# zdule/distributed_learning

Hardware: AMD Instinct MI355X
Metric: images/sec (whole node) ResNet-50 synthetic ImageNet (higher is better)
Workload: dtype bf16

## Files before the change

### csrc/include/dla_kernels.h

```cpp
#pragma once

#include <hip/hip_runtime.h>
#include <stdint.h>

namespace dla {

enum DType : int { kF32 = 0, kBF16 = 1 };

struct SgdEntry {
  float* param;
  const void* grad;
  float* momentum;
  uint16_t* param_bf16;
  int64_t numel;
};

struct SgdParams {
  float lr;
  float momentum;
  float dampening;
  float weight_decay;
  float grad_scale;
  int nesterov;
  int first_step;
// ... 136 lines not shown
                        hipStream_t stream);
void launch_bn_bwd(const void* dy, const void* y, const uint8_t* mask, const void* x, void* dx, void* dres,
                   int64_t M, int C, int dtype, const float* gamma, float* ws, float* part, float* dgamma,
                   float* dbeta, int mask_mode, hipStream_t stream, const float* ext_part = nullptr,
                   int ext_nrb = 0, int64_t ld_dy = 0);

constexpr int kMaxBnGroups = 4;
struct BnGroups {
  int n;
  int begin[kMaxBnGroups + 1];
  const uint16_t* x[kMaxBnGroups];
  uint16_t* y[kMaxBnGroups];
  const uint16_t* dy[kMaxBnGroups];
  int64_t ldy[kMaxBnGroups], lddy[kMaxBnGroups];
  int64_t ldx[kMaxBnGroups], lddx[kMaxBnGroups];
  int ldp[kMaxBnGroups];
  int C[kMaxBnGroups], tpr[kMaxBnGroups], nrb[kMaxBnGroups];
  const float* part[kMaxBnGroups];
  float* wpart[kMaxBnGroups];
  const float* gamma[kMaxBnGroups];
  const float* beta[kMaxBnGroups];
  float* rm[kMaxBnGroups];
  float* rv[kMaxBnGroups];
  float* ws[kMaxBnGroups];
  float eps[kMaxBnGroups], mom[kMaxBnGroups];
  uint16_t* dx[kMaxBnGroups];
  float* dgamma[kMaxBnGroups];
  float* dbeta[kMaxBnGroups];
};
int bn_group_bwd_rows(int64_t M, const int* C, int n);
void launch_bn_group_fwd(BnGroups G, int64_t M, hipStream_t stream);
void launch_bn_group_bwd(BnGroups G, bool ext, int64_t M, hipStream_t stream);

void launch_bn_relu_maxpool_fwd(const void* x, const float* ws, void* y, uint8_t* pos, int N, int H, int W, int C,
                                int OH, int OW, int k, int s, int p, hipStream_t stream);
void launch_bn_relu_maxpool_bwd(const void* dy_pool, const uint8_t* pos, const void* x, void* dx, int N, int H, int W,
                                int C, int OH, int OW, int k, int s, int p, const float* gamma, float* ws, float* part,
                                float* dgamma, float* dbeta, hipStream_t stream);

void launch_maxpool_fwd(const void* x, void* y, uint8_t* pos, int N, int H, int W, int C, int OH, int OW, int k,
                        int s, int p, int dtype, hipStream_t stream);
void launch_maxpool_bwd(const void* dy, const uint8_t* pos, void* dx, int N, int H, int W, int C, int OH, int OW,
                        int k, int s, int p, int dtype, hipStream_t stream);
bool pool_fast_index(int64_t work, int64_t d0, int64_t d1, int64_t d2);
void set_pool3_sep(int rows);
int pool3_strip_rows();
void launch_gap_fwd(const void* x, void* y, int N, int HW, int C, int dtype, hipStream_t stream);
void launch_subsample2(const void* x, void* y, int N, int H, int W, int C, hipStream_t stream);
void launch_gap_bwd(const void* dy, void* dx, int N, int HW, int C, int dtype, hipStream_t stream);

void set_mfma_pipeline(int p);
int mfma_pipeline();
int mfma_pipeline_for(int K);
enum TileCfg : int {
  kTileAuto = 0,
  kTile128x128 = 1,
  kTile128x64 = 2,
  kTile64x64 = 3,
  kTile256x128 = 4,
  kTile256x128w4 = 5,
  kTile128x256w4 = 6,
  kTile256x64 = 7,
  kTile256x256 = 8,
  kTile512x128 = 9
};
int pick_tile(int64_t M, int N, int tile, int K = 0, bool wide_ok = true, bool stats = false);
void set_tile256_min_k_stats(int k);
bool tile256_enabled();
bool tn256_enabled();
inline int tile_bm(int cfg) {
  if (cfg == kTile512x128) return 512;
  return cfg == kTile64x64 ? 64
                           : ((cfg == kTile256x128 || cfg == kTile256x128w4 || cfg == kTile256x64 || cfg == kTile256x256)
                                  ? 256
                                  : 128);
}
inline int tile_bn(int cfg) {
  if (cfg == kTile512x128) return 128;
  return (cfg == kTile128x256w4 || cfg == kTile256x256) ? 256
                                                       : ((cfg == kTile128x128 || cfg == kTile256x128 || cfg == kTile256x128w4) ? 128 : 64);
}
int gemm_nt_stats_rows(int M, int N, int tile = kTileAuto, int K = 0, bool stats_fwd = true);
void set_tile256_min_k(int k);
int gemm_stream_rows(int64_t M, int N, int K, int64_t lda, int64_t ldc, bool b_kmajor, bool add = false,
                     bool bnb = false);
struct BnBwdArgs;
bool launch_gemm_stream(const void* A, int64_t lda, const void* B, int64_t ldb, bool b_kmajor, void* C, int64_t ldc,
                        int M, int N, int K, float* stats, hipStream_t stream, const void* addend = nullptr,
                        int64_t ldd = 0, const uint8_t* addend_mask = nullptr, const BnBwdArgs* bn_bwd = nullptr,
                        const float* apply_ws = nullptr, void* apply_out = nullptr);
void set_gemm_stream(int mode);
bool gemm_direct_ok(int N, int64_t ldc, const void* addend, int64_t ldd);
void launch_gemm_direct(const void* A, int64_t lda, const void* B, int64_t ldb, bool b_kmajor, void* C, int64_t ldc,
                        int M, int N, int K, float* stats, const void* addend, int64_t ldd,
                        const uint8_t* addend_mask, hipStream_t stream);
void set_gemm_direct(int mode);
constexpr int kGemmApplyMaxK = 2048;
bool gemm_apply_ok(int64_t M, int N, int K);
void set_gemm_apply_max_k(int k);
void set_gemm256_direct(int mode);
bool gemm256_direct_enabled();
void set_wgrad_w4(int mode);
int gemm_apply_rows(int64_t M);
void launch_gemm_apply(const void* y, const void* r, const float* ws, const float* ws2, void* out, uint8_t* mask,
                       const void* B, int64_t ldb, void* C, int M, int N, int K, float* stats, hipStream_t stream,
                       void* xs = nullptr, int H = 0, int W = 0);
// ... 83 lines not shown
```

### csrc/include/dla_mfma.h

```cpp
#pragma once

#include "dla_common.h"

namespace dla {
namespace mm {

typedef __bf16 bf16x8_t __attribute__((ext_vector_type(8)));
typedef float f32x4_t __attribute__((ext_vector_type(4)));
typedef short s16x4_t __attribute__((ext_vector_type(4)));

struct FastDiv {
  uint32_t d, m_lo, m_hi;
};
__host__ __device__ inline FastDiv make_fastdiv(uint32_t d) {
  const uint64_t m = ((1ull << 40) + d - 1) / d;
  return FastDiv{d, (uint32_t)m, (uint32_t)(m >> 32)};
}
__device__ __forceinline__ uint32_t fdiv(uint32_t n, const FastDiv& f) {
  return (__umulhi(n, f.m_lo) + n * f.m_hi) >> 8;
}

constexpr int kThreads = 256;
#ifndef DLA_RM_SWIZZLE
#define DLA_RM_SWIZZLE 1
#endif
#ifndef DLA_EPI_SWZ
#define DLA_EPI_SWZ 1
#endif

constexpr int kBK = 64;

#ifndef DLA_EPI_PRELOAD
#define DLA_EPI_PRELOAD 1
#endif
#ifndef DLA_TR_CONCAT
#define DLA_TR_CONCAT 1
#endif

__host__ __device__ constexpr int blocks_per_cu(int BM, int BN, int NT) {
  return (NT == kThreads && BM * BN <= 128 * 128) ? 2 : 1;
}

__device__ __forceinline__ f32x4_t mfma16(const bf16x8_t& a, const bf16x8_t& b, const f32x4_t& c) {
  return __builtin_amdgcn_mfma_f32_16x16x32_bf16(a, b, c, 0, 0, 0);
}

#ifndef DLA_MFMA_SHAPE
#define DLA_MFMA_SHAPE 16
#endif
constexpr int kMS = DLA_MFMA_SHAPE;
constexpr int kKS = 512 / kMS;
constexpr int kAccN = kMS * kMS / 64;
static_assert(kMS == 16 || kMS == 32, "MFMA shape 16 or 32");
// ... 480 lines not shown
    loader_step(pa, k0, 0);
    const uint32_t a_base = lds0 + (uint32_t)((t % NS) * (SA + SB)) * 2u + wofs;
#pragma unroll
    for (int i = 0; i < GA::CH; ++i) glds16(loader_src(pa, i, k0, 0), a_base + (uint32_t)(i * NT * 16));
  };
  auto issue_b = [&](int t) {
    const int k0 = kbeg + t * kBK;
    loader_step(pb, k0, 0);
    const uint32_t b_base = lds0 + (uint32_t)((t % NS) * (SA + SB) + SA) * 2u + wofs;
#pragma unroll
    for (int i = 0; i < GB::CH; ++i) glds16(loader_src(pb, i, k0, 0), b_base + (uint32_t)(i * NT * 16));
  };
#pragma unroll
  for (int p = 0; p < NS - 1; ++p)
    if (p < nk) {
      issue_a(p);
      issue_b(p);
    }
  for (int t = 0; t < nk; ++t) {
    if constexpr (NS == 3) {
      if (t + 1 < nk) vm_wait<L>();
      else vm_wait<0>();
    } else {
      vm_wait<0>();
    }
    asm volatile("s_waitcnt lgkmcnt(0)" ::: "memory");
    __builtin_amdgcn_s_barrier();
    asm volatile("" ::: "memory");
    const bool more = t + NS - 1 < nk;
    if (more) issue_a(t + NS - 1);
    const bf16_t* As = base + (t % NS) * (SA + SB);
    const bf16_t* Bs = As + SA;
    kstep_mfma<BM, BN, NT, LA, LB, kT>(As, Bs, wr, wc, acc, [&] {
      if (more) issue_b(t + NS - 1);
    });
  }
  __syncthreads();
}

template <class L, int W, int NT>
__device__ __forceinline__ void bissue(const L& l, int k0, uint32_t lds) {
  constexpr int CH = TileGeom<W, NT>::CH;
  uint32_t vo[CH];
  if (l.bcheck(k0)) {
#pragma unroll
    for (int i = 0; i < CH; ++i) vo[i] = l.bvoff_chk(i, k0);
  } else {
#pragma unroll
    for (int i = 0; i < CH; ++i) vo[i] = l.bvo[i];
  }
  bglds<CH, NT * 16>(vo, l.bsrd, (uint32_t)__builtin_amdgcn_readfirstlane(l.bsoff(k0)), lds);
}

template <int BM, int BN, int NT, int NS, bool kT = false, class LA, class LB>
__device__ __forceinline__ void mainloop_bglds(const LA& la, const LB& lb, int kbeg, int kend, Acc<BM, BN, NT>& acc,
                                               char* smem) {
  static_assert(NS == 2 || NS == 3, "2 or 3 stages");
  static_assert(LA::kNT == NT && LB::kNT == NT, "loaders built for another block size");
  using GA = TileGeom<BM, NT>;
  using GB = TileGeom<BN, NT>;
  using AC = Acc<BM, BN, NT>;
  constexpr int L = GA::CH + GB::CH;
  constexpr int WM = AC::WM, WN = AC::WN, TM = AC::TM, TN = AC::TN;
  constexpr int SA = BM * kBK, SB = BN * kBK;
  bf16_t* base = reinterpret_cast<bf16_t*>(smem);
  const int wave = threadIdx.x >> 6, wr = wave / AC::WGN, wc = wave % AC::WGN;
  const uint32_t lds0 = lds_addr(smem);
  const uint32_t wofs = (uint32_t)__builtin_amdgcn_readfirstlane(wave * 64 * 16);
  const int nk = (kend - kbeg + kBK - 1) / kBK;
  if (nk <= 0) return;
  LA pa = la;
  LB pb = lb;
  pa.prep();
  pb.prep();
  pa.bprep();
  pb.bprep();
  auto issue_a = [&](int t) {
    const int k0 = kbeg + t * kBK;
    loader_step(pa, k0, 0);
    bissue<LA, BM, NT>(pa, k0, lds0 + (uint32_t)((t % NS) * (SA + SB)) * 2u + wofs);
  };
  auto issue_b = [&](int t) {
    const int k0 = kbeg + t * kBK;
    loader_step(pb, k0, 0);
    bissue<LB, BN, NT>(pb, k0, lds0 + (uint32_t)((t % NS) * (SA + SB) + SA) * 2u + wofs);
  };
#pragma unroll
  for (int p = 0; p < NS - 1; ++p)
    if (p < nk) {
      issue_a(p);
      issue_b(p);
    }
  for (int t = 0; t < nk; ++t) {
    if constexpr (NS == 3) {
      if (t + 1 < nk) vm_wait<L>();
      else vm_wait<0>();
    } else {
      vm_wait<0>();
    }
    asm volatile("s_waitcnt lgkmcnt(0)" ::: "memory");
    __builtin_amdgcn_s_barrier();
    asm volatile("" ::: "memory");
    const bool more = t + NS - 1 < nk;
    if (more) issue_a(t + NS - 1);
    const bf16_t* As = base + (t % NS) * (SA + SB);
    const bf16_t* Bs = As + SA;
    kstep_mfma<BM, BN, NT, LA, LB, kT>(As, Bs, wr, wc, acc, [&] {
      if (more) issue_b(t + NS - 1);
    });
  }
  __syncthreads();
}

template <int PIPE, bool kT = false, int BM, int BN, int NT, class LA, class LB>
__device__ __forceinline__ void run_mainloop(const LA& la, const LB& lb, int kbeg, int kend, Acc<BM, BN, NT>& acc,
                                             char* smem) {
  if constexpr (PIPE == 0) mainloop<BM, BN, NT, kT>(la, lb, kbeg, kend, acc, smem);
  else if constexpr (PIPE >= 6) mainloop_bglds<BM, BN, NT, PIPE - 4, kT>(la, lb, kbeg, kend, acc, smem);
  else if constexpr (PIPE >= 4) mainloop_glds2<BM, BN, NT, PIPE - 2, kT>(la, lb, kbeg, kend, acc, smem);
  else mainloop_glds<BM, BN, NT, PIPE, kT>(la, lb, kbeg, kend, acc, smem);
}

template <int PIPE, int BM, int BN, class LA, class LB>
__host__ __device__ constexpr size_t run_mainloop_lds_bytes() {
  return PIPE == 0 ? mainloop_lds_bytes<BM, BN, LA, LB>()
                   : glds_lds_bytes<BM, BN, (PIPE >= 6 ? PIPE - 4 : (PIPE >= 4 ? PIPE - 2 : PIPE))>();
}

template <int BM, int BN, bool kStats, int NT = kThreads>
__host__ __device__ constexpr size_t epilogue_lds_bytes() {
  return (size_t)BM * (BN + 8) * sizeof(bf16_t) > (size_t)NT * 64 ? (size_t)BM * (BN + 8) * sizeof(bf16_t)
                                                                  : (size_t)NT * 64;
}

template <int BM, int BN, int NT = kThreads>
struct ColStats {
  float s[Acc<BM, BN, NT>::TN], q[Acc<BM, BN, NT>::TN];
  __device__ void zero() {
#pragma unroll
    for (int j = 0; j < Acc<BM, BN, NT>::TN; ++j) s[j] = q[j] = 0.f;
  }
};

struct BnBwdEpi {
  const bf16_t* x;
  int64_t ldx;
  const float* ws;
  const uint8_t* mask;
  int mode;
  float* part;
  const uint8_t* dmask;
  const bf16_t* d2;
  int H, W;
  FastDiv fW, fH;
};

struct RowIdent {
  __device__ __forceinline__ int64_t operator()(int64_t gm) const { return gm; }
};

template <int BM, int BN, bool kStats, bool kEpi = false, int NT = kThreads, class RM = RowIdent>
__device__ __forceinline__ void epilogue_bf16(const Acc<BM, BN, NT>& acc, bf16_t* __restrict__ C, int64_t ldc,
                                              int64_t M, int N, int64_t row0, int col0, ColStats<BM, BN, NT>& st,
                                              const bf16_t* __restrict__ D, int64_t ldd, char* smem,
                                              const BnBwdEpi* epi = nullptr, int bm = 0, RM rowmap = RM()) {
  const BnBwdEpi* bnb = (kEpi && epi && epi->x) ? epi : nullptr;
  const uint8_t* __restrict__ dmask = (kEpi && epi) ? epi->dmask : nullptr;
  const bf16_t* __restrict__ d2 = (kEpi && epi) ? epi->d2 : nullptr;
  using AC = Acc<BM, BN, NT>;
  constexpr int WM = AC::WM, WN = AC::WN, TM = AC::TM, TN = AC::TN;
  static_assert(!DLA_EPI_SWZ || BN >= 32, "the staging XOR needs 4 chunks per row");
  constexpr int LDS_C = DLA_EPI_SWZ ? BN : BN + 8;
  auto cs_off = [](int m, int n) {
    if constexpr (DLA_EPI_SWZ) return m * BN + ((((n >> 3) ^ (((m >> 2) & 1) << 1))) << 3) + (n & 7);
    else return m * (BN + 8) + n;
  };
  (void)LDS_C;
  const int tid = threadIdx.x, lane = tid & 63, wid = tid >> 6, wr = wid / AC::WGN, wc = wid % AC::WGN,
            fr = acc_col(lane);
// ... 342 lines not shown
```

### csrc/kernels/conv.hip

```cpp
#include "dla_common.h"
#include "dla_kernels.h"
#include "dla_knob.h"
#include "dla_mfma.h"

#include <algorithm>
#include <cstdlib>
#include <type_traits>

namespace dla {

using namespace mm;

struct ConvGeom {
  int N, H, W, Cin;
  int OH, OW, Cout;
  int stride;
  FastDiv fOW, fOH;
};

template <int W, bool kFlip, int NT = kThreads>
struct Im2colRowLoader {
  static constexpr bool kKMajor = false;
  static constexpr int kNT = NT;
  static constexpr int CH = TileGeom<W, NT>::CH;
// ... 517 lines not shown
  const int tile = lin % ntiles, split = lin / ntiles;
  const int bm = tile / nbn, bn = tile % nbn;
  const int kbeg = split * k_per_split;
  const int kend = min(P, kbeg + k_per_split);
  const int m0 = bm * BM, n0 = bn * BN;
  const KLoader<BM, NT> la{dy, g.Cout, m0, Mo, kend};
  Im2colKLoader<BN, PIPE != 0, NT> lb{x, g, kend};
  lb.init(n0);
  Acc<BM, BN, NT> acc;
  acc.zero();
  run_mainloop<PIPE>(la, lb, kbeg, kend, acc, smem_raw);
  epilogue_f32<BM, BN, NT>(acc, part + (int64_t)split * Mo * No, Mo, No, m0, n0);
}

static int conv_pipeline(int K, int deep) {
  const int forced = mfma_pipeline();
  if (forced >= 0) return forced;
  static Knob k_conv_pipe = Knob::integer("CONV_PIPE", -1);
  const int env = k_conv_pipe.value();
  return K >= 256 ? (env >= 0 ? env : deep) : 0;
}

static ConvGeom make_geom(int N, int H, int W, int Cin, int Cout, int stride) {
  ConvGeom g;
  g.N = N;
  g.H = H;
  g.W = W;
  g.Cin = Cin;
  g.Cout = Cout;
  g.stride = stride;
  g.OH = (H + 2 - 3) / stride + 1;
  g.OW = (W + 2 - 3) / stride + 1;
  g.fOW = make_fastdiv((uint32_t)g.OW);
  g.fOH = make_fastdiv((uint32_t)g.OH);
  return g;
}

template <int BM, int BN, bool S, int PIPE, int NT>
static void launch_fwd_p(const bf16_t* x, const bf16_t* w, bf16_t* y, const ConvGeom& g, float* stats,
                         hipStream_t stream) {
  const int64_t P = (int64_t)g.N * g.OH * g.OW;
  const int tiles = (int)((P + BM - 1) / BM) * ((g.Cout + BN - 1) / BN);
  const size_t lds =
      std::max(run_mainloop_lds_bytes<PIPE % 100, BM, BN, Im2colRowLoader<BM, false, NT>, RowLoader<BN, NT>>(),
               epilogue_lds_bytes<BM, BN, S, NT>());
  hipLaunchKernelGGL((conv3x3_fwd_kernel<BM, BN, S, PIPE, NT>), dim3(tiles), dim3(NT), lds, stream, x, w, y, g,
                     stats);
}
template <int BM, int BN, bool S, int NTW = kThreads>
static void launch_fwd(const bf16_t* x, const bf16_t* w, bf16_t* y, const ConvGeom& g, float* stats,
                       hipStream_t stream) {
  if constexpr (NTW == 512 && BM * BN > 256 * 128) {
    if (mfma_pipeline() == 2) launch_fwd_p<BM, BN, S, 2, 512>(x, w, y, g, stats, stream);
    else launch_fwd_p<BM, BN, S, 6, 512>(x, w, y, g, stats, stream);
  } else if constexpr (NTW == 512) {
    if (mfma_pipeline() == 7) launch_fwd_p<BM, BN, S, 7, 512>(x, w, y, g, stats, stream);
    else launch_fwd_p<BM, BN, S, 3, 512>(x, w, y, g, stats, stream);
  } else if constexpr (BM * BN > 128 * 128) {
    if (mfma_pipeline() == 2) launch_fwd_p<BM, BN, S, 2, kThreads>(x, w, y, g, stats, stream);
    else launch_fwd_p<BM, BN, S, 3, kThreads>(x, w, y, g, stats, stream);
  } else if (g.Cin % 64 != 0) {
    if (mfma_pipeline_for(9 * g.Cin) == 0) launch_fwd_p<BM, BN, S, 100, kThreads>(x, w, y, g, stats, stream);
    else launch_fwd_p<BM, BN, S, 102, kThreads>(x, w, y, g, stats, stream);
  } else {
    switch (conv_pipeline(9 * g.Cin, 6)) {
      case 0: launch_fwd_p<BM, BN, S, 0, kThreads>(x, w, y, g, stats, stream); break;
      case 3: launch_fwd_p<BM, BN, S, 3, kThreads>(x, w, y, g, stats, stream); break;
      case 4: launch_fwd_p<BM, BN, S, 4, kThreads>(x, w, y, g, stats, stream); break;
      case 6: launch_fwd_p<BM, BN, S, 6, kThreads>(x, w, y, g, stats, stream); break;
      default: launch_fwd_p<BM, BN, S, 2, kThreads>(x, w, y, g, stats, stream); break;
    }
  }
}

static Knob k_tile512 = Knob::on_unless_0("TILE512");
static bool tile512_enabled() { return k_tile512.on(); }

int pick_conv_tile(int64_t P, int N, int tile, int K, bool wide_ok) {
  if (tile == kTileAuto && wide_ok && tile256_enabled() && tile512_enabled() && N == 128 && K >= 1024 &&
      (P + 511) / 512 >= 1024)
    return kTile512x128;
  return pick_tile(P, N, tile, K, wide_ok);
}

int conv3x3_stats_rows(int64_t P, int Cout, int tile, int K, bool wide_ok) {
  const int bm = tile_bm(pick_conv_tile(P, Cout, tile, K, wide_ok));
  return (int)((P + bm - 1) / bm);
}

void launch_conv3x3_fwd(const void* x, const void* w, void* y, int N, int H, int W, int Cin, int Cout, int stride,
                        float* stats, hipStream_t stream, int tile) {
  if (tile == kTileAuto && halo_conv_eligible(Cin, Cout, W, stride, true)) {
    launch_conv3x3_halo(x, w, y, N, H, W, stats, stream);
    return;
  }
  const ConvGeom g = make_geom(N, H, W, Cin, Cout, stride);
  const bf16_t* xp = (const bf16_t*)x;
  const bf16_t* wp = (const bf16_t*)w;
  bf16_t* yp = (bf16_t*)y;
#define DLA_CFW(BM_, BN_, NT_)                                                  \
  if (stats) launch_fwd<BM_, BN_, true, NT_>(xp, wp, yp, g, stats, stream);   \
  else launch_fwd<BM_, BN_, false, NT_>(xp, wp, yp, g, stats, stream);
#define DLA_CF(BM_, BN_) DLA_CFW(BM_, BN_, kThreads)
  switch (pick_conv_tile((int64_t)g.N * g.OH * g.OW, Cout, tile, 9 * Cin, Cin % 64 == 0)) {
    case kTile512x128: DLA_CFW(512, 128, 512) break;
    case kTile256x256: DLA_CFW(256, 256, 512) break;
// ... 180 lines not shown
```

### csrc/kernels/gemm.hip

```cpp
#include <cstdlib>
#include <type_traits>

#include "dla_common.h"
#include "dla_kernels.h"
#include "dla_knob.h"
#include "dla_mfma.h"

namespace dla {

using namespace mm;

template <int BM, int BN, bool kStats, bool kBT, int PIPE, int NT, bool kD = false>
__global__ __launch_bounds__(NT, blocks_per_cu(BM, BN, NT)) void gemm_nt_kernel(const bf16_t* __restrict__ A, int64_t lda,
                                                              const bf16_t* __restrict__ B, int64_t ldb,
                                                              bf16_t* __restrict__ C, int64_t ldc, int M, int N, int K,
                                                              float* __restrict__ stats, const bf16_t* __restrict__ D,
                                                              int64_t ldd, BnBwdEpi bnb) {
  extern __shared__ __attribute__((aligned(16))) char smem_raw[];
  const int nbn = (N + BN - 1) / BN;
  const int tile = xcd_remap(blockIdx.x, gridDim.x);
  const int bm = tile / nbn, bn = tile % nbn;
  const int64_t row0 = (int64_t)bm * BM;
  const int col0 = bn * BN;
  ColStats<BM, BN, NT> st;
// ... 97 lines not shown
    }
  }
}

template <typename T, int SG>
__global__ __launch_bounds__(256) void splitk_reduce_sg_kernel(const float* __restrict__ P, int splits, int64_t n,
                                                               T* __restrict__ out, float scale, int accumulate,
                                                               const bf16_t* __restrict__ D, int64_t ldd, int ncol) {
  auto addend = [&](int64_t i) -> float {
    if (D == nullptr) return 0.f;
    const int64_t r = i / ncol;
    return bf16_to_f32(D[r * ldd + (i - r * ncol)]);
  };
  constexpr int kOpb = 256 / SG;
  __shared__ float4_t red[SG][kOpb];
  const int g = threadIdx.x / kOpb, o = threadIdx.x % kOpb;
  const int64_t nv = n / 4;
  const int64_t v = (int64_t)blockIdx.x * kOpb + o;
  float4_t a0{0.f, 0.f, 0.f, 0.f}, a1 = a0;
  if (v < nv) {
    int k = g;
    for (; k + SG < splits; k += 2 * SG) {
      a0 += reinterpret_cast<const float4_t*>(P + (int64_t)k * n)[v];
      a1 += reinterpret_cast<const float4_t*>(P + (int64_t)(k + SG) * n)[v];
    }
    if (k < splits) a0 += reinterpret_cast<const float4_t*>(P + (int64_t)k * n)[v];
  }
  red[g][o] = a0 + a1;
  __syncthreads();
  if (g == 0 && v < nv) {
    float4_t s = red[0][o];
#pragma unroll
    for (int j = 1; j < SG; ++j) s += red[j][o];
    s *= scale;
#pragma unroll
    for (int j = 0; j < 4; ++j) {
      float r = s[j] + addend(v * 4 + j);
      if (accumulate) r += Cvt<T>::to_f32(out[v * 4 + j]);
      out[v * 4 + j] = Cvt<T>::from_f32(r);
    }
  }
  if (blockIdx.x == 0) {
    for (int64_t i = nv * 4 + threadIdx.x; i < n; i += blockDim.x) {
      float r = 0.f;
      for (int k = 0; k < splits; ++k) r += P[(int64_t)k * n + i];
      r = r * scale + addend(i);
      if (accumulate) r += Cvt<T>::to_f32(out[i]);
      out[i] = Cvt<T>::from_f32(r);
    }
  }
}

static int g_pipe = -1;
void set_mfma_pipeline(int p) { g_pipe = (p == 0 || (p >= 2 && p <= 7)) ? p : -1; }
int mfma_pipeline() { return g_pipe; }
int mfma_pipeline_for(int K) { return g_pipe >= 0 ? g_pipe : (K >= 256 ? 2 : 0); }

template <int BM, int BN, bool S, bool BT, int PIPE, int NT, bool kD = false>
static void launch_nt_p(const bf16_t* A, int64_t lda, const bf16_t* B, int64_t ldb, bf16_t* C, int64_t ldc, int M,
                        int N, int K, float* stats, const bf16_t* D, int64_t ldd, const BnBwdEpi& bnb,
                        hipStream_t stream) {
  const int tiles = ((M + BM - 1) / BM) * ((N + BN - 1) / BN);
  const size_t ab = BT ? run_mainloop_lds_bytes<PIPE, BM, BN, RowLoader<BM, NT>, KLoader<BN, NT>>()
                       : run_mainloop_lds_bytes<PIPE, BM, BN, RowLoader<BM, NT>, RowLoader<BN, NT>>();
  const size_t cs = epilogue_lds_bytes<BM, BN, S, NT>();
  hipLaunchKernelGGL((gemm_nt_kernel<BM, BN, S, BT, PIPE, NT, kD>), dim3(tiles), dim3(NT), std::max(ab, cs), stream, A,
                     lda, B, ldb, C, ldc, M, N, K, stats, D, ldd, bnb);
}

template <int BM, int BN, bool S, bool BT, int NTW = kThreads>
static void launch_nt(const bf16_t* A, int64_t lda, const bf16_t* B, int64_t ldb, bf16_t* C, int64_t ldc, int M,
                      int N, int K, float* stats, const bf16_t* D, int64_t ldd, const BnBwdEpi& bnb,
                      hipStream_t stream) {
  if constexpr (NTW == 512 && BM * BN > 256 * 128) {
    if (mfma_pipeline() == 2) launch_nt_p<BM, BN, S, BT, 2, 512>(A, lda, B, ldb, C, ldc, M, N, K, stats, D, ldd, bnb, stream);
    else launch_nt_p<BM, BN, S, BT, 6, 512>(A, lda, B, ldb, C, ldc, M, N, K, stats, D, ldd, bnb, stream);
  } else if constexpr (NTW == 512) {
    if (mfma_pipeline() == 7) launch_nt_p<BM, BN, S, BT, 7, 512>(A, lda, B, ldb, C, ldc, M, N, K, stats, D, ldd, bnb, stream);
    else launch_nt_p<BM, BN, S, BT, 3, 512>(A, lda, B, ldb, C, ldc, M, N, K, stats, D, ldd, bnb, stream);
  } else if constexpr (BM * BN > 128 * 128) {
    if (mfma_pipeline() == 2) launch_nt_p<BM, BN, S, BT, 2, kThreads>(A, lda, B, ldb, C, ldc, M, N, K, stats, D, ldd, bnb, stream);
    else launch_nt_p<BM, BN, S, BT, 3, kThreads>(A, lda, B, ldb, C, ldc, M, N, K, stats, D, ldd, bnb, stream);
  } else {
    const int pipe = mfma_pipeline() >= 0 ? mfma_pipeline() : (K > 512 ? 2 : 0);
    switch (pipe) {
      case 0: launch_nt_p<BM, BN, S, BT, 0, kThreads>(A, lda, B, ldb, C, ldc, M, N, K, stats, D, ldd, bnb, stream); break;
      case 3: launch_nt_p<BM, BN, S, BT, 3, kThreads>(A, lda, B, ldb, C, ldc, M, N, K, stats, D, ldd, bnb, stream); break;
      case 4: launch_nt_p<BM, BN, S, BT, 4, kThreads>(A, lda, B, ldb, C, ldc, M, N, K, stats, D, ldd, bnb, stream); break;
      case 6: launch_nt_p<BM, BN, S, BT, 6, kThreads>(A, lda, B, ldb, C, ldc, M, N, K, stats, D, ldd, bnb, stream); break;
      default: launch_nt_p<BM, BN, S, BT, 2, kThreads>(A, lda, B, ldb, C, ldc, M, N, K, stats, D, ldd, bnb, stream); break;
    }
  }
}

static Knob k_tile256 = Knob::on_unless_0("TILE256");
bool tile256_enabled() { return k_tile256.on(); }

static int g_tile256_min_k = 1024;
void set_tile256_min_k(int k) { g_tile256_min_k = k > 0 ? k : 1024; }
static Knob k_tile256_min_k_stats = Knob::positive("TILE256_MIN_K_STATS", 256);
void set_tile256_min_k_stats(int k) { k_tile256_min_k_stats.set(k); }

static Knob k_gemm256_direct = Knob::off_unless_1("GEMM256_DIRECT");
void set_gemm256_direct(int mode) { k_gemm256_direct.set(mode); }
bool gemm256_direct_enabled() { return k_gemm256_direct.on(); }

int pick_tile(int64_t M, int N, int tile, int K, bool wide_ok, bool stats) {
  if (tile != kTileAuto) return tile;
  const int min_k = stats ? std::min(g_tile256_min_k, k_tile256_min_k_stats.value()) : g_tile256_min_k;
  if (wide_ok && tile256_enabled() && K >= min_k && N % 256 == 0 && ((M + 255) / 256) * (N / 256) >= 192)
    return kTile256x256;
  return N <= 64 ? kTile128x64 : kTile128x128;
}

int gemm_nt_stats_rows(int M, int N, int tile, int K, bool stats_fwd) {
  const int bm = tile_bm(pick_tile(M, N, tile, K, true, stats_fwd));
  return (M + bm - 1) / bm;
}

void launch_gemm_nt(const void* A, int64_t lda, const void* B, int64_t ldb, void* C, int64_t ldc, int M, int N, int K,
                    float* stats, hipStream_t stream, const void* addend, int64_t ld_addend, bool b_kmajor, int tile,
                    const BnBwdArgs* bn_bwd, const uint8_t* addend_mask, const void* addend2_s2, int H, int W) {
  BnBwdEpi bnb{};
  if (bn_bwd) {
    bnb.x = (const bf16_t*)bn_bwd->x;
    bnb.ldx = bn_bwd->ldx;
    bnb.ws = bn_bwd->ws;
    bnb.mask = bn_bwd->mask;
// ... 191 lines not shown
```

### csrc/nn_bindings.cpp

```cpp
#include <torch/extension.h>
#include <ATen/hip/HIPContext.h>
#include <c10/hip/HIPStream.h>

#include "dla_bindings.h"
#include "dla_kernels.h"
#include "dla_knob.h"
#include "dla_tables.h"

namespace dla {

static void check_span(const at::Tensor& t, const char* what) {
  int64_t last = 0;
  for (int64_t d = 0; d < t.dim(); ++d) last += (t.size(d) - 1) * t.stride(d);
  const int64_t bytes = t.numel() ? (last + 1) * (int64_t)t.element_size() : 0;
  TORCH_CHECK(bytes < (int64_t(1) << 31), what, ": ", bytes,
              " bytes reach the 2 GiB buffer-descriptor range of the native kernels (lower the per-GPU batch)");
}

static void check_act(const at::Tensor& t, const char* what) {
  TORCH_CHECK(t.is_cuda(), what, " must be a GPU tensor");
  TORCH_CHECK(t.dim() == 4 || t.dim() == 2, what, " must be NCHW-shaped (channels_last) or [M, C]");
  const bool ok = t.dim() == 4 ? t.is_contiguous(at::MemoryFormat::ChannelsLast) : t.is_contiguous();
  TORCH_CHECK(ok, what, " must be channels_last (4-D) or contiguous (2-D)");
  TORCH_CHECK(t.size(1) % 8 == 0, what, ": channel count must be a multiple of 8");
// ... 1025 lines not shown
                         current_stream(dy));
  return dx;
}

std::vector<at::Tensor> conv3x3_dgrad_bn(at::Tensor dy, at::Tensor w, c10::optional<at::Tensor> addend,
                                         at::Tensor x_bn, at::Tensor ws, c10::optional<at::Tensor> mask, int64_t mode) {
  at::Tensor dx = dgrad_dx("conv3x3_dgrad_bn", dy, w);
  const int N = (int)dy.size(0), Cout = (int)w.size(0), Cin = (int)w.size(1), H = (int)dy.size(2), W = (int)dy.size(3);
  const void* add = dgrad_addend("conv3x3_dgrad_bn", addend, dx);
  const int64_t P = (int64_t)N * H * W;
  at::Tensor part;
  const BnBwdArgs bnb = make_bn_bwd("conv3x3_dgrad_bn", x_bn, ws, mask, mode, P, Cin,
                                    conv3x3_stats_rows(P, Cin, kTileAuto, 9 * Cout, Cout % 64 == 0), part);
  launch_conv3x3_dgrad(dy.data_ptr(), w.data_ptr(), dx.data_ptr(), N, H, W, Cin, Cout, add, current_stream(dy),
                       kTileAuto, &bnb);
  return {dx, part};
}

at::Tensor conv3x3_wgrad(at::Tensor dy, at::Tensor x, int64_t stride, c10::ScalarType out_dtype) {
  const int out_code = out_dtype_code(out_dtype, "conv3x3_wgrad");
  dy = dy.contiguous(at::MemoryFormat::ChannelsLast);
  TORCH_CHECK(x.is_cuda() && x.dim() == 4 && x.scalar_type() == at::kBFloat16 &&
                  x.is_contiguous(at::MemoryFormat::ChannelsLast) && x.size(1) % 8 == 0,
              "conv3x3_wgrad: x must be bf16 channels_last with Cin % 8 == 0");
  TORCH_CHECK(dy.is_cuda() && dy.scalar_type() == at::kBFloat16 && dy.size(1) % 8 == 0,
              "conv3x3_wgrad: dy must be a bf16 GPU tensor, Cout % 8");
  TORCH_CHECK(x.numel() / x.size(1) < (1 << 24), "conv3x3_wgrad: too many pixels");
  const int N = (int)x.size(0), Cin = (int)x.size(1), H = (int)x.size(2), W = (int)x.size(3), Cout = (int)dy.size(1);
  TORCH_CHECK(dy.size(2) == (H - 1) / stride + 1 && dy.size(3) == (W - 1) / stride + 1, "conv3x3_wgrad: dy shape");
  at::Tensor dw = at::empty({Cout, Cin, 3, 3}, x.options().dtype(out_dtype).memory_format(at::MemoryFormat::ChannelsLast));
  if (halo_wgrad_eligible(Cin, Cout, W, (int)stride) && (int64_t)N * (H + 2) * (W + 2) < (1 << 30)) {
    const int hs = halo_wgrad_splits(N, H, W);
    at::Tensor hpart = at::empty({(int64_t)hs * Cout * 9 * Cin}, x.options().dtype(at::kFloat));
    launch_conv3x3_halo_wgrad(dy.data_ptr(), x.data_ptr(), hpart.data_ptr<float>(), hs, dw.data_ptr(), out_code, N, H, W,
                              current_stream(x));
    return dw;
  }
  const int splits = conv3x3_wgrad_splits(N, H, W, Cin, Cout, (int)stride);
  at::Tensor part = at::empty({(int64_t)splits * Cout * 9 * Cin}, x.options().dtype(at::kFloat));
  launch_conv3x3_wgrad(dy.data_ptr(), x.data_ptr(), part.data_ptr<float>(), splits, dw.data_ptr(), out_code, N, H, W,
                       Cin, Cout, (int)stride, current_stream(x));
  return dw;
}

void bind_nn(pybind11::module& m) {
  m.def("gemm_nt_bn", &gemm_nt_bn, "gemm_nt producing a fused BN's dy plus its backward-reduction partials",
        pybind11::arg("A"), pybind11::arg("B"), pybind11::arg("addend"), pybind11::arg("b_kmajor"),
        pybind11::arg("x_bn"), pybind11::arg("ws"), pybind11::arg("mask"), pybind11::arg("mode"),
        pybind11::arg("addend_mask") = pybind11::none(), pybind11::arg("addend2") = pybind11::none(),
        pybind11::arg("H") = 0, pybind11::arg("W") = 0);
  m.def("conv3x3_dgrad_bn", &conv3x3_dgrad_bn, "3x3 dgrad producing a fused BN's dy plus its backward partials",
        pybind11::arg("dy"), pybind11::arg("w"), pybind11::arg("addend"), pybind11::arg("x_bn"), pybind11::arg("ws"),
        pybind11::arg("mask"), pybind11::arg("mode"));
  m.def("set_mfma_pipeline", &set_mfma_pipeline, "MFMA main loop: 0 register staging, 2/3 LDS-DMA stages, -1 per-shape auto");
  m.def("set_gemm_stream", &set_gemm_stream, "persistent streaming 1x1 GEMM: -1 environment (default on), 0 off, 1 on");
  m.def("set_gemm_persist", &set_gemm_persist, "persistent register-stored 1x1 GEMM: blocks per CU (0 off, -1 env)");
  m.def("set_gemm_direct", &set_gemm_direct, "register-stored 128x128 1x1 GEMM tiles: -1 environment (default off), 0 / 1");
  m.def("gemm_stream_rows", &gemm_stream_rows, "BN-statistics partial rows of the streaming GEMM (0: shape not served)",
        pybind11::arg("M"), pybind11::arg("N"), pybind11::arg("K"), pybind11::arg("lda"), pybind11::arg("ldc"), pybind11::arg("b_kmajor") = false,
        pybind11::arg("add") = false, pybind11::arg("bnb") = false);
  m.def("mfma_pipeline", &mfma_pipeline);
  m.def("set_tile256_min_k_stats", &set_tile256_min_k_stats, "smallest K of the auto 256x256 tiles of statistics forwards (A/B)");
  m.def("set_tile256_min_k", &set_tile256_min_k, "smallest K of the auto 256x256 gemm_nt / conv tiles (A/B; <= 0 default 1024)");
  m.def("set_tn256", &set_tn256, "256x256 weight-gradient tiles: -1 environment (DLA_TN256, default on), 0 off, 1 on");
  m.def("set_splitk_blocks", &set_splitk_blocks, "split-K weight-gradient block target (0 = default / DLA_SPLITK_BLOCKS)");
  m.def("splitk_target_blocks", &splitk_target_blocks);
  m.def("set_bn_red_blocks", &set_bn_red_blocks, "BN reduction-pass block target (0 = default / DLA_BN_RED_BLOCKS)");
  m.def("bn_red_blocks", &bn_red_blocks);
  m.def("conv3x3_fwd", &conv3x3_fwd, "implicit-GEMM 3x3/pad-1 conv forward (NHWC bf16, MFMA)", pybind11::arg("x"),
        pybind11::arg("w"), pybind11::arg("stride") = 1, pybind11::arg("stats") = false, pybind11::arg("tile") = 0);
  m.def("conv3x3_dgrad", &conv3x3_dgrad, "implicit-GEMM 3x3 conv data gradient (stride 1)", pybind11::arg("dy"),
        pybind11::arg("w"), pybind11::arg("addend") = pybind11::none(), pybind11::arg("tile") = 0);
  m.def("conv3x3s2_dgrad", &conv3x3s2_dgrad, "implicit-GEMM 3x3 / stride-2 conv data gradient (parity classes)",
        pybind11::arg("dy"), pybind11::arg("w"), pybind11::arg("H"), pybind11::arg("W"));
  m.def("conv3x3_wgrad", &conv3x3_wgrad, "implicit-GEMM 3x3 conv weight gradient (split-K)", pybind11::arg("dy"),
        pybind11::arg("x"), pybind11::arg("stride") = 1, pybind11::arg("out_dtype") = at::kFloat);
  m.def("bn_relu_maxpool_fwd", &bn_relu_maxpool_fwd, "stem BN(train)+ReLU+max-pool forward (pooled output only)",
        pybind11::arg("x"), pybind11::arg("weight"), pybind11::arg("bias"), pybind11::arg("running_mean"),
        pybind11::arg("running_var"), pybind11::arg("momentum"), pybind11::arg("eps"), pybind11::arg("k"),
        pybind11::arg("s"), pybind11::arg("p"), pybind11::arg("stats") = pybind11::none(),
        pybind11::arg("ceil_mode") = false);
  m.def("bn_relu_maxpool_bwd", &bn_relu_maxpool_bwd, "stem BN+ReLU+max-pool backward (dy gathered from the pool)",
        pybind11::arg("dy_pool"), pybind11::arg("pos"), pybind11::arg("x"), pybind11::arg("ws"), pybind11::arg("weight"),
        pybind11::arg("k"), pybind11::arg("s"), pybind11::arg("p"), pybind11::arg("want_dx") = true);
  m.def("maxpool_fwd", &maxpool_fwd, "NHWC max pooling forward (+ argmax window positions)", pybind11::arg("x"),
        pybind11::arg("k"), pybind11::arg("s"), pybind11::arg("p"), pybind11::arg("ceil_mode") = false,
        pybind11::arg("need_pos") = true);
  m.def("maxpool_bwd", &maxpool_bwd, "NHWC max pooling backward (gather form)");
  m.def("set_pool3_sep", &set_pool3_sep, "3x3/s1 max-pool forward: 4 / 7-row separable strips, 0 generic kernel, -1 environment (default 4)");
  m.def("pool3_strip_rows", &pool3_strip_rows, "strip height of the 3x3/s1 max-pool forward in force (0: generic kernel)");
  m.def("pool_fast_index", &pool_fast_index, "whether a pool kernel over `work` indices with divisors d0, d1, d2 decodes by multiply-shift",
        pybind11::arg("work"), pybind11::arg("d0"), pybind11::arg("d1"), pybind11::arg("d2"));
  m.def("bn_dual_fwd", &bn_dual_fwd, "training act(BN(x) + BN_d(xd)) in one apply pass (downsample residual)",
        pybind11::arg("x"), pybind11::arg("xd"), pybind11::arg("weight"), pybind11::arg("bias"),
        pybind11::arg("running_mean"), pybind11::arg("running_var"), pybind11::arg("weight_d"), pybind11::arg("bias_d"),
        pybind11::arg("running_mean_d"), pybind11::arg("running_var_d"), pybind11::arg("momentum"),
        pybind11::arg("momentum_d"), pybind11::arg("eps"), pybind11::arg("eps_d"), pybind11::arg("relu"),
        pybind11::arg("stats"), pybind11::arg("stats_d"), pybind11::arg("defer") = false);
  m.def("bn_apply_deferred", &bn_apply_deferred, "the apply pass of a deferred bn_act_fwd / bn_dual_fwd (ReLU, residual)",
        pybind11::arg("x"), pybind11::arg("r"), pybind11::arg("ws"), pybind11::arg("wsd"), pybind11::arg("y"),
        pybind11::arg("mask"));
  m.def("gemm_nt_apply", &gemm_nt_apply,
        "1x1-conv forward over a deferred act(BN(y) + r): writes the BN output + mask and returns (C, stats)",
        pybind11::arg("y"), pybind11::arg("r"), pybind11::arg("ws"), pybind11::arg("wsd"), pybind11::arg("B"),
        pybind11::arg("stats"), pybind11::arg("out"), pybind11::arg("mask"), pybind11::arg("xs") = pybind11::none(),
        pybind11::arg("H") = 0, pybind11::arg("W") = 0);
  m.def("gemm_nt_apply_ok", &gemm_nt_apply_ok, "shapes gemm_nt_apply serves (M rows, N outputs, K channels)");
// ... 80 lines not shown
```

### distributed_learning_amd/knobs.py

```python
from __future__ import annotations

import os
from dataclasses import dataclass
from typing import Dict, Optional


@dataclass(frozen=True)
class Knob:
    default: str
    where: str
    what: str


PREFIX = "DLA_"

TABLE: Dict[str, Knob] = {
    "KERNELS": Knob("native", "bench.py", "native | torch: the model's kernels (bench --kernels default)"),
    "PRECISION": Knob("bf16", "bench.py", "bf16 | autocast | fp32 (bench --precision default)"),
    "CONV": Knob("native", "bench.py", "native | miopen 1x1 convolutions (bench --conv default)"),
    "GRAPH": Knob("off", "bench.py", "on | off: HIP-graph capture of the whole step (bench --graph default)"),
    "SAME_DEVICE": Knob("0", "parallel/context.py", "1: every rank on cuda:0 (gloo + IPC transport)"),
    "TRANSPORT": Knob("", "parallel/context.py", "rccl | ipc gradient transport (default rccl; ipc with SAME_DEVICE)"),
    "COMPUTE_STREAM": Knob("default", "bench.py", "high: the training step runs on a high-priority stream, so its "
                                                  "kernels dispatch ahead of the late weight gradients' side stream"),
    "LAUNCH_GROUPS": Knob("1", "parallel/grad_sync.py", "0: fusion off (bucket cap 0) issues one collective launch per "
                                                        "gradient tensor, the reference's semantics (main.py:168-179); 1: "
                                                        "the per-tensor collectives launch in groups (profiles/r5/g04/)"),
    "DEFER_APPLY": Knob("1", "ops/bn_act.py", "1: a bottleneck block's final BN(+residual)+ReLU output is written by the "
                                              "next block's conv1 GEMM (gemm_apply.hip) instead of its own apply pass"),
    "APPLY_MAX_K": Knob("512", "csrc/kernels/gemm_apply.hip", "largest conv1 input width whose deferred block-final "
                                                               "apply the conv1 GEMM writes (<= 2048)"),
    "WGRAD_W4": Knob("0", "csrc/kernels/conv.hip", "1: 128x256 four-wave tiles for the Cout-128 3x3 weight gradients"),
    "DEFER_MID": Knob("0", "models/resnet.py", "1: a bottleneck's bn2+ReLU output is written by conv3's streaming GEMM "
                                              "(gemm_stream.hip kAp) at the short-K stages instead of its own apply pass; measured slower, profiles/r6/g22/"),
    "APPLY_SUBSAMPLE": Knob("1", "ops/conv.py", "1: at a stage transition the fused conv1 apply also writes the stride-2 "
                                                "subsample of the block output (no subsample2 pass)"),
    "AUTOTUNE_BUDGET_S": Knob("90", "parallel/autotune.py", "wall-clock budget of the all-reduce selection at N > 1"),
    "COMM_TIMEOUT_S": Knob("600", "csrc/comm/engine.cpp", "seconds before a collective / IPC barrier is declared dead"),
    "WGRAD_DEFER": Knob("3x3", "ops/conv.py", "3x3 | auto | all | 0: weight gradients on the side stream "
                                              "(profiles/r3/g18_g19_wgrad_defer.md, g47_defer_batch_ab.md; 'all' "
                                              "stalls for seconds at bs1280, profiles/r6/g27/)"),
    "WGRAD_JOIN": Knob("end", "ops/conv.py", "end | conv: where the compute stream joins the side stream"),
    "WGRAD_DEFER_MIN_AI": Knob("200", "ops/conv.py", "WGRAD_DEFER=auto: 1x1 arithmetic-intensity threshold"),
    "BN_EPILOGUE": Knob("0", "ops/conv.py", "1 / stream: BN-backward partials in every / the streaming dgrad "
                                            "GEMM epilogue (profiles/r4/g02/, bn_epilogue_ab_bs512.jsonl)"),
    "STEM_BN": Knob("1", "ops/conv.py", "0: stem BN+ReLU+max-pool backward apply as its own pass, not inside the "
                                        "stem weight gradient (profiles/r5/g11/)"),
    "BN_GROUPED": Knob("1", "ops/inception.py", "0: one BN launch chain per Inception branch (profiles/r3p/)"),
    "FANIN_CAT": Knob("1", "ops/inception.py", "0: three separate fan-in 1x1 GEMMs (profiles/r3y/)"),
    "STEM_STREAM": Knob("0", "csrc/kernels/gemm_stream.hip", "1: the stem forward (with BN statistics) on the persistent "
                                                             "streaming GEMM instead of the 128x64 tile kernel"),
    "GEMM256_DIRECT": Knob("0", "csrc/kernels/gemm.hip", "1: the 256x256 statistics forwards store their tile and "
                                                          "statistics from registers (dla_mfma.h epilogue_direct)"),
    "TILE256": Knob("1", "csrc/kernels/gemm.hip", "0: no 256x256 tiles for fwd / dgrad (profiles/r5a/)"),
    "TILE512": Knob("1", "csrc/kernels/conv.hip", "0: no 512x128 tiles for the Cout-128 3x3 fwd / dgrad (profiles/r5/g54/)"),
    "TILE256_MIN_K_STATS": Knob("256", "csrc/kernels/gemm.hip", "smallest K of the 256x256 tiles for the forward GEMMs "
                                                                  "with BN statistics (profiles/r6/g11/)"),
    "TN256": Knob("1", "csrc/kernels/gemm.hip", "0: no 256x256 weight-gradient tiles (profiles/r5c/, r5d/)"),
    "SPLITK_XCD": Knob("1", "csrc/kernels/gemm.hip", "0: no XCD-aware split-K grids (round-2 README row)"),
    "SPLITK_BLOCKS": Knob("512", "csrc/kernels/gemm.hip", "split-K grid target in blocks"),
    "SPLITK_SG": Knob("1", "csrc/kernels/gemm.hip", "0: no split-group split-K reduce (profiles/r3n/)"),
    "GEMM_SPLITK": Knob("1", "csrc/nn_bindings.cpp", "0: no split-K for the FC heads"),
    "GEMM_DIRECT": Knob("0", "csrc/kernels/gemm_direct.hip", "1: 128x128 1x1 GEMM tiles stored straight from the "
                                                             "registers, not staged through LDS (neutral: profiles/r6/g03/)"),
    "GEMM_PERSIST": Knob("0", "csrc/kernels/gemm_direct.hip", "n > 0: the register-stored 128x128 tiles (GEMM_DIRECT=1) as a "
                                                              "persistent kernel with n blocks per CU"),
    "GEMM_STREAM": Knob("1", "csrc/kernels/gemm_stream.hip", "0: no persistent streaming 1x1 GEMM (profiles/r3/)"),
    "CONV_PIPE": Knob("-1", "csrc/kernels/conv.hip", "3x3 conv main-loop pipeline for K >= 256 (-1: per shape)"),
    "HALO": Knob("2", "csrc/kernels/conv_halo.hip", "0 off, 1 dgrad only, 2 fwd + dgrad halo-tiled 64-ch 3x3 (r5l/)"),
    "HALO_V": Knob("3", "csrc/kernels/conv_halo.hip", "halo kernel version (1 / 2 / 3 = 2 forward + 1 data "
                                                    "gradient, profiles/r6/g32/)"),
    "HALO_FASTDIV": Knob("1", "csrc/kernels/conv_halo.hip", "0: integer divisions for the halo conv's per-strip tap masks "
                                                            "(A/B of the multiply-shift form, profiles/r6/g30/)"),
    "HALO_DIRECT": Knob("1", "csrc/kernels/conv_halo.hip", "1: the variant-1 halo data gradient stores its tile from "
                                                           "registers (transposed product) instead of through LDS "
                                                           "(profiles/r6/g34/)"),
    "HALO_DIRECT_FWD": Knob("0", "csrc/kernels/conv_halo.hip", "1: the variant-2 halo forward stores its tile and "
                                                               "statistics from registers"),
    "HALO_WGRAD": Knob("1", "csrc/kernels/conv_halo_wgrad.hip", "0: implicit-GEMM 64-ch 3x3 weight gradient"),
    "POOL3_SEP": Knob("4", "csrc/kernels/pool.hip", "separable 3x3 stride-1 max-pool variant (4 / 7; other: off; r3w/; set_pool3_sep)"),
    "BN_RED_BLOCKS": Knob("1024", "csrc/kernels/bn_act.hip", "BN reduction-pass block target"),
    "HOOK_TIMING": Knob("0", "parallel/grad_sync.py", "1: host time inside the gradient hooks"),
    "TRACE": Knob("0", "utils/trace.py", "1: roctx ranges per phase"),
    "VERBOSE": Knob("", "utils/log.py", "log level (default INFO)"),
    "TORCH_PROF": Knob("", "bench.py", "path: torch.profiler table after the timed region"),
    "AUTOBUILD": Knob("0", "ops/_ext.py", "1: build the extension on first import"),
    "EXT_SO": Knob("", "ops/_ext.py", "path of a variant _C.so (A/B builds, _build.py --out)"),
    "ALLOW_STALE": Knob("0", "ops/_ext.py", "1: load a _C.so whose embedded source digest differs from csrc/"),
}

_CACHE: Dict[str, str] = {}


def get(name: str) -> str:
    if name not in TABLE:
        raise KeyError(f"unknown knob {name!r}; every switch must be listed in knobs.TABLE")
    if name not in _CACHE:
        _CACHE[name] = os.environ.get(PREFIX + name, TABLE[name].default)
    return _CACHE[name]


def flag(name: str) -> bool:
    return get(name) not in ("", "0", "off", "false", "False")


def env_name(name: str) -> str:
    return PREFIX + name


def non_default(environ: Optional[Dict[str, str]] = None) -> Dict[str, str]:
# ... 20 lines not shown
```

Baseline: 15970.

## Add ping-pong quadrant main loop for 256x256 8-wave MFMA tiles

Adds a new PIPE 8 main loop for the 256x256 512-thread tiles with row-major operands. It splits each k-tile into four MFMA quadrants, interleaving LDS fragment loads and half-tile buffer DMA issues between them, and staggers the two wave halves by one barrier so one group computes while the other loads. It is enabled by default for 3x3 forward convs and for non-transposed 1x1 GEMMs with K >= 1024, through a new TILE256_LOOP knob. The aim is to hide LDS and global load latency behind MFMA work, at the cost of a more intricate barrier schedule and higher register pressure.

```diff
diff --git a/csrc/include/dla_kernels.h b/csrc/include/dla_kernels.h
--- a/csrc/include/dla_kernels.h
+++ b/csrc/include/dla_kernels.h
@@ -212,6 +212,7 @@
 void set_mfma_pipeline(int p);
 int mfma_pipeline();
 int mfma_pipeline_for(int K);
+bool tile256_loop8(int K, int min_k_auto = 0);
 enum TileCfg : int {
   kTileAuto = 0,
   kTile128x128 = 1,
diff --git a/csrc/include/dla_mfma.h b/csrc/include/dla_mfma.h
--- a/csrc/include/dla_mfma.h
+++ b/csrc/include/dla_mfma.h
@@ -1,4 +1,6 @@
 #pragma once
+
+#include <type_traits>
 
 #include "dla_common.h"
 
@@ -585,6 +587,20 @@
   bglds<CH, NT * 16>(vo, l.bsrd, (uint32_t)__builtin_amdgcn_readfirstlane(l.bsoff(k0)), lds);
 }
 
+template <class L, int W, int NT, int H>
+__device__ __forceinline__ void bissue_half(const L& l, int k0, uint32_t lds) {
+  static_assert(TileGeom<W, NT>::CH == 4 && (H == 0 || H == 1), "two half-tiles of two slots");
+  uint32_t vo[2];
+  if (l.bcheck(k0)) {
+#pragma unroll
+    for (int i = 0; i < 2; ++i) vo[i] = l.bvoff_chk(2 * H + i, k0);
+  } else {
+#pragma unroll
+    for (int i = 0; i < 2; ++i) vo[i] = l.bvo[2 * H + i];
+  }
+  bglds<2, NT * 16>(vo, l.bsrd, (uint32_t)__builtin_amdgcn_readfirstlane(l.bsoff(k0)), lds + (uint32_t)(2 * H * NT * 16));
+}
+
 template <int BM, int BN, int NT, int NS, bool kT = false, class LA, class LB>
 __device__ __forceinline__ void mainloop_bglds(const LA& la, const LB& lb, int kbeg, int kend, Acc<BM, BN, NT>& acc,
                                                char* smem) {
@@ -645,10 +661,122 @@
   __syncthreads();
 }
 
+constexpr int kPipe8MinKSteps = 4;
+
+template <int I0, int J0, bool kT, int KK, int HM, int HN, class AC>
+__device__ __forceinline__ void quadrant_mfma(AC& acc, const bf16x8_t (&af)[KK][HM], const bf16x8_t (&bfr)[KK][HN]) {
+  asm volatile("s_waitcnt lgkmcnt(0)" ::: "memory");
+  __builtin_amdgcn_sched_barrier(0);
+  __builtin_amdgcn_s_setprio(1);
+#pragma unroll
+  for (int kk = 0; kk < KK; ++kk)
+#pragma unroll
+    for (int i = 0; i < HM; ++i)
+#pragma unroll
+      for (int j = 0; j < HN; ++j) acc.v[I0 + i][J0 + j] = mfma_t<kT>(af[kk][i], bfr[kk][j], acc.v[I0 + i][J0 + j]);
+  __builtin_amdgcn_s_setprio(0);
+  __builtin_amdgcn_sched_barrier(0);
+  __builtin_amdgcn_s_barrier();
+}
+
+template <int BM, int BN, int NT, bool kT = false, class LA, class LB>
+__device__ __forceinline__ void mainloop_bglds8(const LA& la, const LB& lb, int kbeg, int kend, Acc<BM, BN, NT>& acc,
+                                                char* smem) {
+  static_assert(BM == 256 && BN == 256 && NT == 512, "PIPE 8 is the 256 x 256 8-wave tile's loop");
+  static_assert(!LA::kKMajor && !LB::kKMajor, "PIPE 8 stages row-major operand images only");
+  static_assert(LA::kNT == NT && LB::kNT == NT, "loaders built for another block size");
+  using GA = TileGeom<BM, NT>;
+  using GB = TileGeom<BN, NT>;
+  using AC = Acc<BM, BN, NT>;
+  static_assert(AC::WGM == 4 && AC::WGN == 2 && AC::TM % 2 == 0 && AC::TN % 2 == 0, "4 x 2 waves, even fragment counts");
+  static_assert(GA::CH == 4 && GB::CH == 4, "two DMA instructions per thread per half-tile");
+  constexpr int WM = AC::WM, WN = AC::WN, HM = AC::TM / 2, HN = AC::TN / 2, KK = kBK / kKS;
+  constexpr int SA = BM * kBK, SB = BN * kBK;
+  bf16_t* base = reinterpret_cast<bf16_t*>(smem);
+  const int wave = threadIdx.x >> 6, wr = wave / AC::WGN, wc = wave % AC::WGN;
+  const bool late = __builtin_amdgcn_readfirstlane(wr >= AC::WGM / 2) != 0;
+  const uint32_t lds0 = lds_addr(smem);
+  const uint32_t wofs = (uint32_t)__builtin_amdgcn_readfirstlane(wave * 64 * 16);
+  const int nk = (kend - kbeg + kBK - 1) / kBK;
+  if (nk <= 0) return;
+  LA pa = la;
+  LB pb = lb;
+  pa.prep();
+  pb.prep();
+  pa.bprep();
+  pb.bprep();
+  auto issue_a = [&](int t) {
+    const int k0 = kbeg + t * kBK;
+    loader_step(pa, k0, 0);
+    bissue<LA, BM, NT>(pa, k0, lds0 + (uint32_t)((t & 1) * (SA + SB)) * 2u + wofs);
+  };
+  auto issue_b = [&](int t) {
+    const int k0 = kbeg + t * kBK;
+    loader_step(pb, k0, 0);
+    bissue<LB, BN, NT>(pb, k0, lds0 + (uint32_t)((t & 1) * (SA + SB) + SA) * 2u + wofs);
+  };
+  auto issue_bh = [&](int t, auto half) {
+    const int k0 = kbeg + t * kBK;
+    loader_step(pb, k0, 0);
+    bissue_half<LB, BN, NT, decltype(half)::value>(pb, k0, lds0 + (uint32_t)((t & 1) * (SA + SB) + SA) * 2u + wofs);
+  };
+  bf16x8_t a0[KK][HM], a1[KK][HM], bq[KK][HN];
+  auto ktile = [&](int u, int par) {
+    const bf16_t* As = base + par * (SA + SB);
+    const bf16_t* Bs = As + SA;
+#pragma unroll
+    for (int kk = 0; kk < KK; ++kk)
+#pragma unroll
+      for (int i = 0; i < HM; ++i) a0[kk][i] = glds_frag<BM, LA>(As, wr * WM + i * kMS, kk);
+    __builtin_amdgcn_sched_barrier(0);
+#pragma unroll
+    for (int kk = 0; kk < KK; ++kk)
+#pragma unroll
+      for (int j = 0; j < HN; ++j) bq[kk][j] = glds_frag<BN, LB>(Bs, wc * WN + j * kMS, kk);
+    issue_bh(u + 1, std::integral_constant<int, 0>{});
+    __builtin_amdgcn_s_barrier();
+    quadrant_mfma<0, 0, kT>(acc, a0, bq);
+#pragma unroll
+    for (int kk = 0; kk < KK; ++kk)
+#pragma unroll
+      for (int i = 0; i < HM; ++i) a1[kk][i] = glds_frag<BM, LA>(As, wr * WM + (HM + i) * kMS, kk);
+    issue_bh(u + 1, std::integral_constant<int, 1>{});
+    __builtin_amdgcn_s_barrier();
+    quadrant_mfma<HM, 0, kT>(acc, a1, bq);
+#pragma unroll
+    for (int kk = 0; kk < KK; ++kk)
+#pragma unroll
+      for (int j = 0; j < HN; ++j) bq[kk][j] = glds_frag<BN, LB>(Bs, wc * WN + (HN + j) * kMS, kk);
+    __builtin_amdgcn_s_barrier();
+    quadrant_mfma<HM, HN, kT>(acc, a1, bq);
+    issue_a(u + 2);
+    vm_wait<GA::CH>();
+    __builtin_amdgcn_s_barrier();
+    quadrant_mfma<0, HN, kT>(acc, a0, bq);
+  };
+  issue_a(0);
+  issue_b(0);
+  issue_a(1);
+  vm_wait<GA::CH>();
+  __builtin_amdgcn_s_barrier();
+  asm volatile("" ::: "memory");
+  if (late) __builtin_amdgcn_s_barrier();
+  int u = 0;
+  for (; u + 1 < nk; u += 2) {
+    ktile(u, 0);
+    ktile(u + 1, 1);
+  }
+  if (u < nk) ktile(u, 0);
+  if (!late) __builtin_amdgcn_s_barrier();
+  vm_wait<0>();
+  __syncthreads();
+}
+
 template <int PIPE, bool kT = false, int BM, int BN, int NT, class LA, class LB>
 __device__ __forceinline__ void run_mainloop(const LA& la, const LB& lb, int kbeg, int kend, Acc<BM, BN, NT>& acc,
                                              char* smem) {
   if constexpr (PIPE == 0) mainloop<BM, BN, NT, kT>(la, lb, kbeg, kend, acc, smem);
+  else if constexpr (PIPE == 8) mainloop_bglds8<BM, BN, NT, kT>(la, lb, kbeg, kend, acc, smem);
   else if constexpr (PIPE >= 6) mainloop_bglds<BM, BN, NT, PIPE - 4, kT>(la, lb, kbeg, kend, acc, smem);
   else if constexpr (PIPE >= 4) mainloop_glds2<BM, BN, NT, PIPE - 2, kT>(la, lb, kbeg, kend, acc, smem);
   else mainloop_glds<BM, BN, NT, PIPE, kT>(la, lb, kbeg, kend, acc, smem);
@@ -657,7 +785,7 @@
 template <int PIPE, int BM, int BN, class LA, class LB>
 __host__ __device__ constexpr size_t run_mainloop_lds_bytes() {
   return PIPE == 0 ? mainloop_lds_bytes<BM, BN, LA, LB>()
-                   : glds_lds_bytes<BM, BN, (PIPE >= 6 ? PIPE - 4 : (PIPE >= 4 ? PIPE - 2 : PIPE))>();
+                   : glds_lds_bytes<BM, BN, (PIPE == 8 ? 2 : PIPE >= 6 ? PIPE - 4 : (PIPE >= 4 ? PIPE - 2 : PIPE))>();
 }
 
 template <int BM, int BN, bool kStats, int NT = kThreads>
diff --git a/csrc/kernels/conv.hip b/csrc/kernels/conv.hip
--- a/csrc/kernels/conv.hip
+++ b/csrc/kernels/conv.hip
@@ -593,6 +593,7 @@
                        hipStream_t stream) {
   if constexpr (NTW == 512 && BM * BN > 256 * 128) {
     if (mfma_pipeline() == 2) launch_fwd_p<BM, BN, S, 2, 512>(x, w, y, g, stats, stream);
+    else if (BM == 256 && BN == 256 && tile256_loop8(9 * g.Cin)) launch_fwd_p<256, 256, S, 8, 512>(x, w, y, g, stats, stream);
     else launch_fwd_p<BM, BN, S, 6, 512>(x, w, y, g, stats, stream);
   } else if constexpr (NTW == 512) {
     if (mfma_pipeline() == 7) launch_fwd_p<BM, BN, S, 7, 512>(x, w, y, g, stats, stream);
diff --git a/csrc/kernels/gemm.hip b/csrc/kernels/gemm.hip
--- a/csrc/kernels/gemm.hip
+++ b/csrc/kernels/gemm.hip
@@ -173,9 +173,15 @@
 }
 
 static int g_pipe = -1;
-void set_mfma_pipeline(int p) { g_pipe = (p == 0 || (p >= 2 && p <= 7)) ? p : -1; }
+void set_mfma_pipeline(int p) { g_pipe = (p == 0 || (p >= 2 && p <= 8)) ? p : -1; }
 int mfma_pipeline() { return g_pipe; }
 int mfma_pipeline_for(int K) { return g_pipe >= 0 ? g_pipe : (K >= 256 ? 2 : 0); }
+
+static Knob k_tile256_loop = Knob::integer("TILE256_LOOP", 8);
+bool tile256_loop8(int K, int min_k_auto) {
+  if ((K + kBK - 1) / kBK < kPipe8MinKSteps) return false;
+  return g_pipe >= 0 ? g_pipe == 8 : (k_tile256_loop.value() == 8 && K >= min_k_auto);
+}
 
 template <int BM, int BN, bool S, bool BT, int PIPE, int NT, bool kD = false>
 static void launch_nt_p(const bf16_t* A, int64_t lda, const bf16_t* B, int64_t ldb, bf16_t* C, int64_t ldc, int M,
@@ -195,6 +201,7 @@
                       hipStream_t stream) {
   if constexpr (NTW == 512 && BM * BN > 256 * 128) {
     if (mfma_pipeline() == 2) launch_nt_p<BM, BN, S, BT, 2, 512>(A, lda, B, ldb, C, ldc, M, N, K, stats, D, ldd, bnb, stream);
+    else if (!BT && tile256_loop8(K, 1024)) launch_nt_p<BM, BN, S, false, 8, 512>(A, lda, B, ldb, C, ldc, M, N, K, stats, D, ldd, bnb, stream);
     else launch_nt_p<BM, BN, S, BT, 6, 512>(A, lda, B, ldb, C, ldc, M, N, K, stats, D, ldd, bnb, stream);
   } else if constexpr (NTW == 512) {
     if (mfma_pipeline() == 7) launch_nt_p<BM, BN, S, BT, 7, 512>(A, lda, B, ldb, C, ldc, M, N, K, stats, D, ldd, bnb, stream);
diff --git a/csrc/nn_bindings.cpp b/csrc/nn_bindings.cpp
--- a/csrc/nn_bindings.cpp
+++ b/csrc/nn_bindings.cpp
@@ -1101,7 +1101,11 @@
   m.def("conv3x3_dgrad_bn", &conv3x3_dgrad_bn, "3x3 dgrad producing a fused BN's dy plus its backward partials",
         pybind11::arg("dy"), pybind11::arg("w"), pybind11::arg("addend"), pybind11::arg("x_bn"), pybind11::arg("ws"),
         pybind11::arg("mask"), pybind11::arg("mode"));
-  m.def("set_mfma_pipeline", &set_mfma_pipeline, "MFMA main loop: 0 register staging, 2/3 LDS-DMA stages, -1 per-shape auto");
+  m.def("set_mfma_pipeline", &set_mfma_pipeline, "MFMA main loop: 0 register staging, 2/3 LDS-DMA stages, 4/5 the v2 LDS-DMA schedule, 6/7 buffer-DMA stages, "
+        "8 the 256x256 ping-pong loop (other tiles keep their default), -1 per-shape auto");
+  m.def("tile256_loop8", &tile256_loop8, py::arg("K"), py::arg("min_k_auto") = 0,
+        "whether the 256x256 row-major-operand tiles run the ping-pong loop at this K (min_k_auto: the family's threshold "
+        "when no loop is forced; gemm_nt uses 1024)");
   m.def("set_gemm_stream", &set_gemm_stream, "persistent streaming 1x1 GEMM: -1 environment (default on), 0 off, 1 on");
   m.def("set_gemm_persist", &set_gemm_persist, "persistent register-stored 1x1 GEMM: blocks per CU (0 off, -1 env)");
   m.def("set_gemm_direct", &set_gemm_direct, "register-stored 128x128 1x1 GEMM tiles: -1 environment (default off), 0 / 1");
diff --git a/distributed_learning_amd/knobs.py b/distributed_learning_amd/knobs.py
--- a/distributed_learning_amd/knobs.py
+++ b/distributed_learning_amd/knobs.py
@@ -56,6 +56,9 @@
     "TILE512": Knob("1", "csrc/kernels/conv.hip", "0: no 512x128 tiles for the Cout-128 3x3 fwd / dgrad (profiles/r5/g54/)"),
     "TILE256_MIN_K_STATS": Knob("256", "csrc/kernels/gemm.hip", "smallest K of the 256x256 tiles for the forward GEMMs "
                                                                   "with BN statistics (profiles/r6/g11/)"),
+    "TILE256_LOOP": Knob("8", "csrc/kernels/gemm.hip", "6: the 256x256 tiles with row-major operands (3x3 forward, 1x1 "
+                                                         "forward) keep the lockstep buffer-DMA loop instead of the "
+                                                         "ping-pong loop (profiles/mainloop8/)"),
     "TN256": Knob("1", "csrc/kernels/gemm.hip", "0: no 256x256 weight-gradient tiles (profiles/r5c/, r5d/)"),
     "SPLITK_XCD": Knob("1", "csrc/kernels/gemm.hip", "0: no XCD-aware split-K grids (round-2 README row)"),
     "SPLITK_BLOCKS": Knob("512", "csrc/kernels/gemm.hip", "split-K grid target in blocks"),
```

Result: no change. 15850 (-0.7%).
